# HKUST-Aerial-Robotics/Omni-swarm

Measured on AMD Instinct MI355X. Metric: keyframes/sec (4x fisheye 600x480) + p50 loop-match ms @ 100k-frame DB, higher is better.
Workload: dtype f16

## Files before the change

omni-swarm_amd/csrc/config.h:

```cpp
#pragma once
#include "common.h"

namespace omni {

enum CfgId {
    CFG_CONV_V1 = 0, CFG_RS_TRN, CFG_DET16, CFG_SP_SPARSE_DESC, CFG_SP_SPARSE_DA, CFG_SP_FUSED_CAND, CFG_SP_SPLIT_DB, CFG_SP_MASK_SKIP, CFG_SP_MASK_SKIP_SPLIT, CFG_SP_MASK_RECT, CFG_SPLIT_FUSE1A, CFG_SPLIT_WINO,
    CFG_SPLIT_TRN, CFG_CONV_XCD, CFG_SP_PROFILE_MASK, CFG_PP_U8, CFG_PP_TRACE, CFG_PP_DBG, CFG_RS_TRACE, CFG_SPLIT_TRACE, CFG_SPLIT_DBG, CFG_WINO_TRACE, CFG_ROCTX,
    CFG_VLAD_BIG, CFG_VLAD_STEM_FUSE, CFG_VLAD_UNFUSED, CFG_VLAD_MFMA, CFG_VLAD_SBLOCK, CFG_VLAD_MBLOCK_PX, CFG_VLAD_MFMA_PX, CFG_VLAD_FC_MFMA, CFG_VLAD_MBLOCK_CPW,
    CFG_VLAD_SB_LDSPAD, CFG_VLAD_SB_PERSIST, CFG_VLAD_SB_TRACE, CFG_VLAD_SB_DBG, CFG_VLAD_MASK_SKIP,
    CFG_SCAN_ROWS_MIN, CFG_MQ_ROT, CFG_MQ_MIN, CFG_INDEX_MIRROR, CFG_INDEX_MIRROR_MIN_ROWS, CFG_INDEX_CERT_FAIL,
    CFG_GEOMETRY_THREADS, CFG_MESSAGE_THREADS, CFG_GEOMETRY_ASYNC, CFG_DETECTOR_ASYNC, CFG_PIPELINE_ONE_STREAM, CFG_PIPELINE_FIFO, CFG_PIPELINE_UNIT_PLAN,
    CFG_JPEGDEC_SUBSEQ_BITS, CFG_JPEGDEC_RESTART_WGS, CFG_JPEGDEC_PLAIN_WGS, CFG_JPEGDEC_UNSTUFF_DEV,
    CFG_HW_QUEUES,
    CFG_RCCL_LIB,
    CFG_COUNT
};
enum CfgClass {
    CFG_VARIANT = 0,
    CFG_TUNING = 1,
    CFG_DEBUG = 2,
    CFG_TEST = 3,
    CFG_STRING = 4
};
struct CfgOption { const char* env; int def, lo, hi; int cls; const char* doc; };
// ... 13 lines not shown
```

omni-swarm_amd/csrc/config.hip:

```cpp
#include "config.h"
#include "stream_plan.h"

#include <atomic>
#include <cerrno>
#include <climits>
#include <cstdlib>

namespace omni {

const CfgOption kCfgOptions[CFG_COUNT] = {
    {"OMNI_CONV_V1", 0, 0, 3, CFG_VARIANT, "fp16 3x3 layers: 0 = production (conv1a fused into the ping-pong conv1b, register-stationary cin=128); 1 = generic kernel, 2 = persistent LDS-DMA kernel, "
                                           "3 = ping-pong without the conv1a fusion -- 1-3 exist only in the test build of the library (lib_test/)"},
    {"OMNI_RS_TRN", -1, -1, 1, CFG_VARIANT, "register-stationary kernel of the unpooled cin=128 fp16 layers: tile orientation, -1 = the one with fewer tiles, 0 = plain, 1 = transposed"},
    {"OMNI_DET16", 1, 0, 1, CFG_VARIANT, "detector head of the fp16 and OMNI_PREC_SPLIT paths on v_mfma_f32_32x32x16_f16 with split (hi, lo) operands (0: the exact-f32 MFMA kernel)"},
    {"OMNI_SP_SPARSE_DESC", 1, 0, 1, CFG_VARIANT, "convDb + descriptor norm only at the cells around the key points (0: dense descriptor map)"},
    {"OMNI_SP_SPARSE_DA", 1, 0, 1, CFG_VARIANT, "convDa only at those cells too (fp16 and OMNI_PREC_SPLIT; 0: dense convDa)"},
    {"OMNI_SP_FUSED_CAND", 1, 0, 1, CFG_VARIANT, "getKeyPoints' threshold inside the detector head's epilogue + window masks from the candidate list (0: sp_cand_kernel re-reads the heat map)"},
    {"OMNI_SP_SPLIT_DB", 1, 0, 1, CFG_VARIANT, "OMNI_PREC_SPLIT: convDb + descriptor norm at the key points' cells with split (hi, lo) operands on the fp16 matrix cores (0: exact-f32 MFMA convolution)"},
    {"OMNI_SP_MASK_SKIP", 1, 0, 1, CFG_VARIANT, "fp16: the tile rows inside the image-independent band of the fisheye mask are left out of the tile walk (0: every tile)"},
    {"OMNI_SP_MASK_SKIP_SPLIT", 1, 0, 1, CFG_VARIANT, "the same for OMNI_PREC_SPLIT"},
    {"OMNI_SP_MASK_RECT", 0, 0, 1, CFG_TEST, "1: a masked pass leaves out only the rectangle of tiles where the output is one constant vector, filled by broadcasting that vector "
                                             "(what was skipped before the band: the A/B reference, same results)"},
    {"OMNI_SPLIT_FUSE1A", 1, 0, 1, CFG_VARIANT, "OMNI_PREC_SPLIT: conv1a built inside the conv1b kernel from the u8 image (0: separate exact-f32 conv1a pass)"},
    {"OMNI_SPLIT_WINO", 7, 0, 15, CFG_VARIANT, "OMNI_PREC_SPLIT: the cin = 64 layers as Winograd F(2x2,3x3) kernels with split operands (conv_wino.hip), bit 0 = conv1b (with the conv1a "
                                                "fusion), 1 = conv2a, 2 = conv2b, 3 = conv3a (off by default: same time as the direct kernel, profiles/r06g); 0: the direct kernels of conv_split.hip"},
    {"OMNI_SPLIT_TRN", -1, -1, 1, CFG_VARIANT, "OMNI_PREC_SPLIT cin=128 kernel: tile orientation, as OMNI_RS_TRN"},
    {"OMNI_CONV_XCD", 1, 0, 1, CFG_VARIANT, "persistent convolution kernels derive (cout group, tile walk) from an XCD-aware block id: the cout groups of a pixel tile and its neighbours "
                                           "share one L2 (0: plain blockIdx; process-wide, same results either way)"},
    {"OMNI_SP_PROFILE_MASK", 0, 0, 1, CFG_TUNING, "omni_sp_profile times the stages with the fisheye mask on (what the key-frame pipeline runs)"},
    {"OMNI_PP_U8", 1, 0, 1, CFG_VARIANT, "fp16 conv1a inside conv1b's kernel: matrix-core operands straight from the image bytes (0: through the 256-entry u8 -> (hi, lo) table in LDS)"},
    {"OMNI_PP_TRACE", 0, 0, 1, CFG_DEBUG, "s_memtime trace of the ping-pong conv kernel on stderr"},
    {"OMNI_PP_DBG", 0, 0, 255, CFG_DEBUG, "ping-pong conv kernel timing ablations (WRONG results)"},
    {"OMNI_RS_TRACE", 0, 0, 1, CFG_DEBUG, "s_memtime trace of the register-stationary kernel"},
    {"OMNI_SPLIT_TRACE", 0, 0, 1, CFG_DEBUG, "s_memtime trace of the split-precision kernel"},
    {"OMNI_SPLIT_DBG", 0, 0, 3, CFG_DEBUG, "split-precision kernel timing ablations: 1 = no stores, 2 = every DMA reads tile 0 (WRONG results)"},
    {"OMNI_WINO_TRACE", 0, 0, 1, CFG_DEBUG, "s_memtime trace of the Winograd split kernel"},
    {"OMNI_ROCTX", 0, 0, 1, CFG_DEBUG, "roctx ranges around upload / SuperPoint / MobileNetVLAD / post-processing / BF match / index add + search / exchange and the host loop's "
                                      "stages (rocprofv3 --marker-trace; the library is resolved by dlopen)"},
    {"OMNI_VLAD_BIG", 0, 0, 128, CFG_TUNING, "64 / 128: the 64- / 128-pixel tiles of the unfused block kernel (measured slower at 600x480)"},
    {"OMNI_VLAD_STEM_FUSE", 1, 0, 1, CFG_VARIANT, "stem + block 0 in one kernel (0: two kernels)"},
    {"OMNI_VLAD_UNFUSED", 0, 0, 1, CFG_VARIANT, "1: every block as expand / depthwise / project launches"},
    {"OMNI_VLAD_MFMA", 1, 0, 1, CFG_VARIANT, "late blocks' 1x1 convolutions on the matrix cores"},
    {"OMNI_VLAD_SBLOCK", 1, 0, 1, CFG_VARIANT, "fused split-fp16 block kernel (vlad_s.hip)"},
    {"OMNI_VLAD_MBLOCK_PX", 2048, 0, 1 << 24, CFG_TUNING, "fused matrix-core block kernel for blocks of at most this many input pixels per image (0 disables)"},
    {"OMNI_VLAD_MFMA_PX", 0, 0, 1 << 24, CFG_TUNING, "> 0: matrix-core 1x1 convolutions for blocks of at most this many input pixels per image (default 2048)"},
// ... 138 lines not shown
```

omni-swarm_amd/csrc/conv.h:

```cpp
#pragma once
#include "common.h"
#include "tile_walk.h"

namespace omni {

#define CONV_TH 8
#define CONV_TW 32
#define RS_TH 6
#define RS_TW 32
int conv_rs_pool_tile_rows();
#define CONV_COUT_TILE 64
#define CONV_CIN_CHUNK 64

static inline size_t conv_packed_elems(int cin, int cout, int ksize) { return (size_t)cin * cout * ksize * ksize; }

void conv_pack_weights_f16(const float* w_oihw, int cin, int cout, int ksize, __half* out);
void conv_pack_weights_f32(const float* w_oihw, int cin, int cout, int ksize, float* out);

struct ConvArgs {
    const void* in;
    void* out;
    const void* w_packed;
    const float* bias;
    int batch, H, W, cin, cout, ksize;
// ... 23 lines not shown
void conv1a_split_pack_fused(const float* w , const float* bias , uint16_t* frag );
int conv1ab_split_fused(hipStream_t stream, const ConvArgs& a, const uint8_t* gray, int gstride, int fisheye_mask, const void* w1a_frag, const uint32_t* lut_hl);
float conv_pack_weights_wino(const float* w_oihw, int cin, int cout, uint16_t* out);
int conv_wino(hipStream_t stream, const ConvArgs& a, bool out_split);
int conv1ab_wino_fused(hipStream_t stream, const ConvArgs& a, const uint8_t* gray, int gstride, int fisheye_mask, const void* w1a_frag, const uint32_t* lut_hl, bool out_split);
int split_to_raw32(hipStream_t stream, const void* in_split, void* out_raw, int batch, int C, int H, int W);
int conv_read_pixels2x2_bytes(hipStream_t stream, const void* map, int64_t row_bytes, int64_t org_bytes, int pix_bytes, int y, int x, void* vec);
int conv_fill_rect2x2_bytes(hipStream_t stream, void* map, int batch, int64_t img_bytes, int64_t row_bytes, int64_t org_bytes, int pix_bytes, int y0, int y1, int x0, int x1,
                            const void* vec);
int raw32_to_nchw_f32(hipStream_t stream, const void* in_raw, float* out, int batch, int C, int H, int W);
__host__ __device__ inline int split_frame_w(int W) { return ((W + 31) & ~31) + 2; }
__host__ __device__ inline int split_frame_h(int H) { return ((H + 31) & ~31) + 2; }
inline size_t split_frame_bytes(int H, int W, int C) { return (size_t)split_frame_h(H) * split_frame_w(W) * C * 4; }

int conv1ab_fused(hipStream_t stream, const ConvArgs& a, const uint8_t* gray, int gstride, int fisheye_mask, const _Float16* w1a_frag,
                  const float* bias1a, const uint32_t* lut_hl);
void conv1a_pack_split_weights(const float* w , const float* bias , uint16_t* frag );
void conv1a_make_split_lut(uint32_t* lut );
void conv1a_pack_u8_weights(const float* w , const float* bias , uint16_t* frag );

int conv1a_direct(hipStream_t stream, int precision, const uint8_t* gray, int stride, int batch, int H, int W,
                  int fisheye_mask, const float* w, const float* bias, const float* u8_lut, void* out);

int detector_head(hipStream_t stream, int precision, const void* in, int in_stride, int in_off, int batch, int Hc, int Wc,
                  const float* wT, const float* bias, float* semi);

#if defined(__HIPCC__)
__device__ __forceinline__ int xcd_block_id(int enable) {
    const int n = (int)gridDim.x, b = (int)blockIdx.x;
    return (enable && (n & 7) == 0) ? (b & 7) * (n >> 3) + (b >> 3) : b;
}
// ... 31 lines not shown
```

omni-swarm_amd/csrc/conv.hip:

```cpp
#include "config.h"
#include "conv.h"
#include <type_traits>

namespace omni {

typedef _Float16 half8_t __attribute__((ext_vector_type(8)));
typedef _Float16 half4_t __attribute__((ext_vector_type(4)));
typedef float floatx16 __attribute__((ext_vector_type(16)));
typedef float floatx4 __attribute__((ext_vector_type(4)));

template <typename T, int KG, int EPL>
static void pack_weights(const float* w, int cin, int cout, int ks, T* out) {
    const int taps = ks * ks, n_ct = cout / 64, n_ch = cin / 64;
    size_t o = 0;
    for (int ct = 0; ct < n_ct; ++ct)
        for (int ch = 0; ch < n_ch; ++ch)
            for (int tap = 0; tap < taps; ++tap)
                for (int kg = 0; kg < KG; ++kg)
                    for (int m = 0; m < 2; ++m)
                        for (int l = 0; l < 64; ++l)
                            for (int e = 0; e < EPL; ++e) {
                                const int co = ct * 64 + m * 32 + (l & 31);
                                const int ci = ch * 64 + kg * (64 / KG) + (l >> 5) * EPL + e;
                                const float v = w[((size_t)co * cin + ci) * taps + tap];
// ... 394 lines not shown
        const uint32_t addr = bb[ky + (WHICH == 3 ? 1 : 0)][kx] ^ (kg << 5);
        asm volatile("ds_read_b128 %0, %1" : "=v"(dst) : "v"(addr));
    } else {
        constexpr int aoff = (STEP % 18) * 2048 + (WHICH == 2 ? 1024 : 0);
        const uint32_t ab = STEP < 18 ? a_base0 : a_base1;
        asm volatile("ds_read_b128 %0, %1 offset:%2" : "=v"(dst) : "v"(ab), "i"(aoff));
    }
}
template <int STEP>
__device__ __forceinline__ void pp_load_step(uint32_t a_base0, uint32_t a_base1, const uint32_t (&bb)[4][3], half8_t& fa0, half8_t& fa1,
                                             half8_t& fb0, half8_t& fb1) {
    pp_read<STEP, 0>(a_base0, a_base1, bb, fb0);
    pp_read<STEP, 1>(a_base0, a_base1, bb, fa0);
    pp_read<STEP, 2>(a_base0, a_base1, bb, fa1);
    pp_read<STEP, 3>(a_base0, a_base1, bb, fb1);
}

template <int N>
__device__ __forceinline__ void pp_wait(half8_t& fa0, half8_t& fa1, half8_t& fb0, half8_t& fb1) {
    asm volatile("s_waitcnt lgkmcnt(%4)" : "+v"(fa0), "+v"(fa1), "+v"(fb0), "+v"(fb1) : "i"(N));
}

template <int STEP, int ABL>
__device__ __forceinline__ void pp_mfma_steps(uint32_t a_base0, uint32_t a_base1, const uint32_t (&bb)[4][3], floatx16 (&acc)[2][2],
                                              half8_t (&fa0)[3], half8_t (&fa1)[3], half8_t (&fb0)[3], half8_t (&fb1)[3]) {
    if constexpr (STEP < 36) {
        constexpr int sl = STEP % 3, nx = (STEP + 2) % 3;
        constexpr bool pre = STEP + 2 < 36;
        constexpr bool rdB = pre && ABL != 1 && ABL != 2, rdA = pre && ABL != 1 && ABL != 3;
        pp_wait<ABL ? 0 : ((STEP + 1 < 36) ? 4 : 0)>(fa0[sl], fa1[sl], fb0[sl], fb1[sl]);
// ... 17 lines not shown
        pp_mfma_steps<STEP + 1, ABL>(a_base0, a_base1, bb, acc, fa0, fa1, fb0, fb1);
    }
}

struct Fuse1aArgs {
    const uint8_t* gray; int gstride; int mask_r0, mask_r1;
    const _Float16* w1a_frag;
    const float* bias1a;
    const uint32_t* lut_hl;
    unsigned long long* trace;
    const char* zero_page;
    uint32_t magic_tpi;
    TileWalk walk;
};

template <bool POOL, int ABL, bool FUSE1A>
__global__ void __launch_bounds__(PP_THREADS)
conv3x3_c64_pp_kernel(const _Float16* __restrict__ in, _Float16* __restrict__ out, const _Float16* __restrict__ wp,
                      const float* __restrict__ bias, int H, int W, int cout, int n_ct, int tiles_x, int tiles_y, int batch, int relu, int dbg,
                      Fuse1aArgs fz) {
    extern __shared__ __attribute__((aligned(16))) char smem_raw[];
    const uint32_t lds0 = (uint32_t)(uintptr_t)(__attribute__((address_space(3))) char*)smem_raw;
    const int tid = threadIdx.x, lane = tid & 63;
    const int wave = __builtin_amdgcn_readfirstlane(tid >> 6);
    const int grp = wave >> 2, wl = wave & 3;
    const int n = lane & 31, hh = lane >> 5;
    const int bid = xcd_block_id(fz.walk.xcd);
    const int ct = bid % n_ct, wg = bid / n_ct, nwg = gridDim.x / n_ct;
    const int total = batch * fz.walk.act;
    const int n_mine = wg < total ? (total - wg + nwg - 1) / nwg : 0;

    {
        const uint4* src = reinterpret_cast<const uint4*>(wp + (int64_t)ct * 9 * 4096);
        uint4* dst = reinterpret_cast<uint4*>(smem_raw);
        for (int i = tid; i < C64_W_BYTES / 16; i += PP_THREADS) dst[i] = src[i];
    }
    constexpr int BUFB = FUSE1A ? C64_PIX * 128 : C64_BUF_BYTES;
    char* const buf = smem_raw + C64_W_BYTES + grp * BUFB;
    const uint32_t buf_lds = lds0 + C64_W_BYTES + grp * BUFB;
    uint32_t bb[4][3];
#pragma unroll
    for (int r = 0; r < 4; ++r)
#pragma unroll
        for (int kx = 0; kx < 3; ++kx) {
            const int p = (2 * wl + r) * C64_ITW + n + kx;
            bb[r][kx] = buf_lds + p * 128 + ((hh ^ ((p >> 1) & 7)) << 4);
        }
    const uint32_t a_base0 = lds0 + lane * 16, a_base1 = a_base0 + 18 * 2048;

    auto tile_origin = [&](int t, int& b, int& ty0, int& tx0) {
        b = tile_walk_div(t, fz.magic_tpi);
        int ry, rx;
        tile_walk_rc(fz.walk, tiles_x, t - b * fz.walk.act, ry, rx);
        ty0 = ry * CONV_TH; tx0 = rx * CONV_TW;
// ... 56 lines not shown
        const int p = (3 * wl + fi) * 32 + n;
        fr_iy[fi] = p / C64_ITW; fr_ix[fi] = p - fr_iy[fi] * C64_ITW;
    }
    unsigned char* const patch = reinterpret_cast<unsigned char*>(lut_lds + 256) + wl * 240;
    int tap_off[5];
#pragma unroll
    for (int k = 0; k < 5; ++k) { const int tp = hh ? (k < 4 ? 5 + k : 8) : k; tap_off[k] = (tp / 3) * 40 + tp % 3; }
    auto build_issue = [&](int b, int ty0, int tx0, uint32_t& pv) {
        const int j = lane / 10, d = lane - j * 10;
        int yy = ty0 - 2 + fr_r0 + j, xo = ((tx0 - 2) & ~3) + 4 * d;
        yy = yy < 0 ? 0 : (yy >= H ? H - 1 : yy);
        xo = xo < 0 ? 0 : (xo > fz.gstride - 4 ? fz.gstride - 4 : xo);
        const auto rsrc = __builtin_amdgcn_make_buffer_rsrc(const_cast<uint8_t*>(fz.gray), 0, batch * H * fz.gstride, 0x00020000);
        pv = __builtin_amdgcn_raw_buffer_load_b32(rsrc, (b * H + yy) * fz.gstride + xo, 0, 0);
    };
    auto build_finish = [&](int b, int ty0, int tx0, uint32_t pv, unsigned long long* stamp = nullptr) {
        (void)b;
        const int cx0 = (tx0 - 2) & ~3, xsh = (tx0 - 2) - cx0;
        {
            const int j = lane / 10, d = lane - j * 10;
            const int yy = ty0 - 2 + fr_r0 + j, x0c = cx0 + 4 * d;
            const bool rok = yy >= 0 && yy < H && !(yy >= fz.mask_r0 && yy < fz.mask_r1);
            uint32_t bm = 0;
#pragma unroll
            for (int k = 0; k < 4; ++k) bm |= (x0c + k >= 0 && x0c + k < W) ? (0xFFu << (8 * k)) : 0u;
            if (lane < 60) reinterpret_cast<uint32_t*>(patch)[lane] = rok ? (pv & bm) : 0u;
        }
        half8_t wa[2][2];
#pragma unroll
        for (int j = 0; j < 2; ++j)
#pragma unroll
// ... 33 lines not shown
        for (int fi = 0; fi < 3; ++fi) {
            if (fi >= nf) continue;
#pragma unroll
            for (int m = 0; m < 2; ++m) {
#pragma unroll
                for (int i = 0; i < 16; ++i) a1[fi][m][i] = 0.f;
                a1[fi][m] = __builtin_amdgcn_mfma_f32_32x32x16_f16(wa[0][m], B0[fi], a1[fi][m], 0, 0, 0);
            }
        }
#pragma unroll
        for (int fi = 0; fi < 3; ++fi) {
            if (fi >= nf) continue;
#pragma unroll
            for (int m = 0; m < 2; ++m) a1[fi][m] = __builtin_amdgcn_mfma_f32_32x32x16_f16(wa[1][m], B1[fi], a1[fi][m], 0, 0, 0);
        }
        __builtin_amdgcn_s_setprio(0);
        if (stamp) stamp[1] = __builtin_amdgcn_s_memtime();
#pragma unroll
        for (int fi = 0; fi < 3; ++fi) {
            if (fi >= nf) continue;
            const int p = (3 * wl + fi) * 32 + n;
            const uint32_t sw = (uint32_t)((p >> 1) & 7);
            char* const prow = buf + p * 128 + 8 * hh;
            if (p < C64_PIX) {
#pragma unroll
                for (int m = 0; m < 2; ++m)
#pragma unroll
                    for (int gq = 0; gq < 4; ++gq)
                        *reinterpret_cast<uint2*>(prow + (((uint32_t)(m * 4 + gq) ^ sw) << 4)) =
                            make_uint2(pack_relu_f16(a1[fi][m][4 * gq + 0], a1[fi][m][4 * gq + 1], 1), pack_relu_f16(a1[fi][m][4 * gq + 2], a1[fi][m][4 * gq + 3], 1));
            }
        }
    };

    int k_load = grp;
    int ob = 0, oty0 = 0, otx0 = 0;
    __syncthreads();
    if (grp == 0 && k_load < n_mine) {
        tile_origin(wg + k_load * nwg, ob, oty0, otx0);
        if constexpr (FUSE1A) {
            uint32_t pv;
            build_issue(ob, oty0, otx0, pv);
            build_finish(ob, oty0, otx0, pv);
        } else {
            issue(ob, oty0, otx0);
            asm volatile("s_waitcnt vmcnt(0)" ::: "memory");
        }
        k_load += 2;
    }
    __syncthreads();

    floatx16 acc[2][2];
    int t_pending = -1;
    for (int p = 0; p <= n_mine; ++p) {
        if ((p & 1) == grp) {
            if (p < n_mine) {
#pragma unroll
                for (int m = 0; m < 2; ++m)
#pragma unroll
                    for (int f = 0; f < 2; ++f)
#pragma unroll
                        for (int i = 0; i < 16; ++i) acc[m][f][i] = 0.f;
#pragma unroll
                for (int r = 0; r < 4; ++r)
#pragma unroll
                    for (int kx = 0; kx < 3; ++kx) asm volatile("" : "+v"(bb[r][kx]));
                half8_t fa0[3], fa1[3], fb0[3], fb1[3];
                pp_load_step<0>(a_base0, a_base1, bb, fa0[0], fa1[0], fb0[0], fb1[0]);
                pp_load_step<1>(a_base0, a_base1, bb, fa0[1], fa1[1], fb0[1], fb1[1]);
                __builtin_amdgcn_sched_barrier(0);
                if (!(dbg & 16)) __builtin_amdgcn_s_setprio(2);
                const bool trc = fz.trace && blockIdx.x == 0 && wl == 0 && lane == 0 && p >= 2 && p < 6;
                if (trc) fz.trace[p * 8 + 4] = __builtin_amdgcn_s_memtime();
                pp_mfma_steps<0, ABL>(a_base0, a_base1, bb, acc, fa0, fa1, fb0, fb1);
                if (trc) fz.trace[p * 8 + 5] = __builtin_amdgcn_s_memtime();
                __builtin_amdgcn_s_setprio(0);
                t_pending = wg + p * nwg;
            }
        } else {
            float4 bs[POOL ? 1 : 2][4];
            if constexpr (POOL) bias4(n & 1, bs[0]);
            else { bias4(0, bs[0]); bias4(1, bs[1]); }
            __builtin_amdgcn_sched_barrier(0);
            const bool load = k_load < n_mine && !(dbg & 1);
            if (dbg & 32) __builtin_amdgcn_s_setprio(3);
            uint32_t pv = 0;
            const bool tr = fz.trace && blockIdx.x == 0 && wl == 0 && lane == 0 && p >= 2 && p < 6;
            if (tr) fz.trace[p * 8 + 0] = __builtin_amdgcn_s_memtime();
            int nb = 0, nty0 = 0, ntx0 = 0;
            if (load) {
                tile_origin(wg + k_load * nwg, nb, nty0, ntx0);
                if constexpr (FUSE1A) build_issue(nb, nty0, ntx0, pv);
                else issue(nb, nty0, ntx0);
            }
            if (tr) fz.trace[p * 8 + 1] = __builtin_amdgcn_s_memtime();
            bool full = false;
            if (t_pending >= 0 && !(dbg & 2)) {
                const int b = ob, ty0 = oty0, tx0 = otx0;
                full = (ty0 + CONV_TH <= H) && (tx0 + CONV_TW <= W);
                const int ox = tx0 + n;
                if constexpr (POOL) {
                    const int oy = ty0 + 2 * wl;
                    const bool odd = n & 1;
                    float v[16], q0[16], q1[16];
#pragma unroll
                    for (int i = 0; i < 16; ++i) { q0[i] = vmax(acc[0][0][i], acc[0][1][i]); q1[i] = vmax(acc[1][0][i], acc[1][1][i]); }
                    __builtin_amdgcn_sched_barrier(0);
#pragma unroll
                    for (int i = 0; i < 16; ++i) {
                        const float h0 = vmax_swap_pairs(q0[i]), h1 = vmax_swap_pairs(q1[i]);
                        v[i] = odd ? h1 : h0;
                    }
// ... 5 lines not shown
                        const int oy = ty0 + 2 * wl + f;
#pragma unroll
                        for (int m = 0; m < 2; ++m) {
                            float v[16];
#pragma unroll
                            for (int i = 0; i < 16; ++i) v[i] = acc[m][f][i];
                            _Float16* o = out + (((int64_t)b * H + oy) * W + ox) * cout + ct * 64 + m * 32;
                            store_frag16<false>(v, bs[m], o, hh, relu, (oy < H) && (ox < W));
                        }
                    }
                }
                t_pending = -1;
            }
            if (tr) fz.trace[p * 8 + 2] = __builtin_amdgcn_s_memtime();
            if (load && FUSE1A) {
                if constexpr (FUSE1A) build_finish(nb, nty0, ntx0, pv, tr ? fz.trace + p * 8 + 6 : nullptr);
                if (tr) fz.trace[p * 8 + 3] = __builtin_amdgcn_s_memtime();
                k_load += 2;
                ob = nb; oty0 = nty0; otx0 = ntx0;
            } else if (load) {
                if (full) {
                    if constexpr (POOL) asm volatile("s_waitcnt vmcnt(2)" ::: "memory");
                    else asm volatile("s_waitcnt vmcnt(8)" ::: "memory");
                } else {
                    asm volatile("s_waitcnt vmcnt(0)" ::: "memory");
                }
                if (tr) fz.trace[p * 8 + 3] = __builtin_amdgcn_s_memtime();
                k_load += 2;
                ob = nb; oty0 = nty0; otx0 = ntx0;
            }
        }
        if (dbg & 32) __builtin_amdgcn_s_setprio(0);
        asm volatile("s_waitcnt lgkmcnt(0)" ::: "memory");
        __builtin_amdgcn_s_barrier();
    }
}

template <bool POOL, int ABL, bool FUSE1A = false>
static int launch_conv_pp_abl(hipStream_t st, const ConvArgs& a, int n_cu, int dbg, const Fuse1aArgs& fz = Fuse1aArgs{}) {
    auto kfn = conv3x3_c64_pp_kernel<POOL, ABL, FUSE1A>;
    constexpr int smem_bytes = FUSE1A ? PP_SMEM_FUSED : PP_SMEM;
    static_assert(smem_bytes <= 160 * 1024, "LDS budget");
    OMNI_HIP_TRY(hipFuncSetAttribute((const void*)kfn, hipFuncAttributeMaxDynamicSharedMemorySize, smem_bytes));
    const int tiles_x = cdiv(a.W, CONV_TW), tiles_y = cdiv(a.H, CONV_TH), n_ct = a.cout / 64;
    Fuse1aArgs fzz = fz;
    if (int rc = tile_walk_plan(fzz.walk, "conv", tiles_x, tiles_y, a.skip_ty0, a.skip_ty1, a.skip_tx0, a.skip_tx1)) return rc;
    fzz.walk.xcd = config_process()[CFG_CONV_XCD];
    const int total = a.batch * fzz.walk.act;
    const int per_ct = tile_walk_grid(n_cu, n_ct, cdiv(total, 2));
    OMNI_REQUIRE(a.zero_page, OMNI_ERR_INVALID, "conv: ConvArgs.zero_page is not set");
    fzz.zero_page = reinterpret_cast<const char*>(a.zero_page);
    OMNI_REQUIRE((int64_t)total * (tiles_x * tiles_y) < (1ll << 32), OMNI_ERR_INVALID, "conv: too many tiles for the multiply-high division");
    fzz.magic_tpi = tile_walk_magic(fzz.walk.act);
    static const bool want_trace = config_process()[CFG_PP_TRACE] != 0;
    static unsigned long long* trace_dev = nullptr;
    if (want_trace && !FUSE1A) {
        if (!trace_dev) OMNI_HIP_TRY(hipMalloc((void**)&trace_dev, 64 * 8));
        OMNI_HIP_TRY(hipMemsetAsync(trace_dev, 0, 64 * 8, st));
        fzz.trace = trace_dev;
    }
    hipLaunchKernelGGL(kfn, dim3(per_ct * n_ct), dim3(PP_THREADS), smem_bytes, st, reinterpret_cast<const _Float16*>(a.in),
                       reinterpret_cast<_Float16*>(a.out), reinterpret_cast<const _Float16*>(a.w_packed), a.bias, a.H, a.W, a.cout, n_ct,
                       tiles_x, tiles_y, a.batch, a.relu ? 1 : 0, dbg, fzz);
    OMNI_LAUNCH_CHECK();
    if (want_trace && !FUSE1A) {
        unsigned long long h[64];
        OMNI_HIP_TRY(hipMemcpyAsync(h, trace_dev, sizeof(h), hipMemcpyDeviceToHost, st));
        OMNI_HIP_TRY(hipStreamSynchronize(st));
        static int launches = 0;
        if (total >= 16 * per_ct && launches++ < 2)
            for (int p = 2; p < 6; ++p)
                if (h[p * 8])
                    fprintf(stderr, "pp trace pool=%d H=%d W=%d cout=%d phase %d: service: issue %llu epilogue %llu dma wait %llu | partner mfma loop %llu\n", (int)POOL, a.H, a.W,
                            a.cout, p, h[p * 8 + 1] - h[p * 8], h[p * 8 + 2] - h[p * 8 + 1], h[p * 8 + 3] - h[p * 8 + 2], h[(p ^ 1) * 8 + 5] - h[(p ^ 1) * 8 + 4]);
    }
    return OMNI_OK;
// ... 582 lines not shown
}

template <typename T, int KS, bool POOL>
static int launch_conv(hipStream_t st, const ConvArgs& a) {
    const size_t smem = conv_smem_bytes<T, KS>();
    auto kfn = conv_mfma_kernel<T, KS, POOL>;
    OMNI_HIP_TRY(hipFuncSetAttribute((const void*)kfn, hipFuncAttributeMaxDynamicSharedMemorySize, (int)smem));
    dim3 grid(cdiv(a.W, CONV_TW) * cdiv(a.H, CONV_TH), a.cout / CONV_COUT_TILE, a.batch);
    hipLaunchKernelGGL(kfn, grid, dim3(256), smem, st, reinterpret_cast<const T*>(a.in), a.out, reinterpret_cast<const T*>(a.w_packed),
                       a.bias, a.H, a.W, a.cin, a.cout, a.relu ? 1 : 0, a.out_f32 ? 1 : 0, a.in_cstride > 0 ? a.in_cstride : a.cin);
    OMNI_LAUNCH_CHECK();
    return OMNI_OK;
}

int conv1ab_fused(hipStream_t st, const ConvArgs& a, const uint8_t* gray, int gstride, int fisheye_mask, const _Float16* w1a_frag,
                  const float* bias1a, const uint32_t* lut_hl) {
    OMNI_REQUIRE(a.cin == 64 && a.cout % 64 == 0 && a.ksize == 3 && a.pool && a.n_cu > 0, OMNI_ERR_INVALID, "conv1ab_fused: bad layer shape");
    OMNI_REQUIRE(gstride % 4 == 0 && ((uintptr_t)gray & 3) == 0 && (int64_t)a.batch * a.H * gstride < (1ll << 31), OMNI_ERR_INVALID,
                 "conv1ab_fused: image rows must be 4-byte aligned (stride %d)", gstride);
    Fuse1aArgs fz;
    fz.gray = gray; fz.gstride = gstride;
    omni_fisheye_mask_rows(a.H, fisheye_mask, &fz.mask_r0, &fz.mask_r1);
    fz.w1a_frag = w1a_frag; fz.bias1a = bias1a; fz.lut_hl = lut_hl; fz.trace = nullptr;
    static const bool want_trace = config_process()[CFG_PP_TRACE] != 0;
    static unsigned long long* trace_dev = nullptr;
    if (want_trace) {
        if (!trace_dev) OMNI_HIP_TRY(hipMalloc((void**)&trace_dev, 64 * 8));
        OMNI_HIP_TRY(hipMemsetAsync(trace_dev, 0, 64 * 8, st));
        fz.trace = trace_dev;
    }
    static const int dbg = config_process()[CFG_PP_DBG];
    const int rc = launch_conv_pp_abl<true, 0, true>(st, a, a.n_cu, dbg, fz);
    if (want_trace && rc == OMNI_OK) {
        unsigned long long h[64];
        OMNI_HIP_TRY(hipMemcpyAsync(h, trace_dev, sizeof(h), hipMemcpyDeviceToHost, st));
        OMNI_HIP_TRY(hipStreamSynchronize(st));
        static int printed = 0;
        if (printed++ == 20)
            for (int p = 2; p < 6; ++p)
                fprintf(stderr, "pp trace phase %d: service start %llu issue +%llu epilogue +%llu build +%llu (operands ready +%llu, first fragment +%llu) | mfma loop %llu cycles (start +%lld vs service start)\n", p,
                        h[p * 8], h[p * 8 + 1] - h[p * 8], h[p * 8 + 2] - h[p * 8 + 1], h[p * 8 + 3] - h[p * 8 + 2], h[p * 8 + 6] - h[p * 8 + 2], h[p * 8 + 7] - h[p * 8 + 6],
                        h[p * 8 + 5] - h[p * 8 + 4], (long long)(h[p * 8 + 4] - h[p * 8]));
    }
    return rc;
}

static inline uint16_t f2h_bits(float v) { const __half h = __float2half_rn(v); uint16_t u; memcpy(&u, &h, 2); return u; }
static inline float h2f(uint16_t u) { __half h; memcpy(&h, &u, 2); return __half2float(h); }
void conv1a_pack_split_weights(const float* w, const float* bias, uint16_t* frag ) {
    for (int j = 0; j < 2; ++j)
        for (int m = 0; m < 2; ++m)
            for (int l = 0; l < 64; ++l)
                for (int e = 0; e < 8; ++e) {
                    const int co = m * 32 + (l & 31), hh = l >> 5;
                    auto hi = [&](int t) { return f2h_bits(w[co * 9 + t]); };
                    auto lo = [&](int t) { return f2h_bits(w[co * 9 + t] - h2f(f2h_bits(w[co * 9 + t]))); };
                    uint16_t v = 0;
// ... 938 lines not shown
```

omni-swarm_amd/csrc/sp_plan.h:

```cpp
#pragma once
#include "../../include/omni_hip.h"

namespace omni {

struct SpHandleFacts {
    int precision = OMNI_PREC_F32, H = 0, W = 0;
    int conv_variant = 0;
    bool det16 = true;
    bool fused_cand = true;
    bool sparse_desc = true;
    bool sparse_da = true;
    bool split_fuse1a = true;
    bool split_db = true;
    int wino = 0;
    bool mask_skip = false;
};

inline int sp_wino_layers(int precision, int requested, int H, int W, bool split_fuse1a) {
    if (precision != OMNI_PREC_SPLIT) return 0;
    int m = requested;
    if (H % 8 != 0 || W % 8 != 0) m &= 7;
    if (H % 4 != 0 || W % 4 != 0) m &= 1;
    if (H % 2 != 0 || W % 2 != 0 || !split_fuse1a) m &= ~1;
    return m;
}

struct SpPassInputs {
// ... 13 lines not shown
    SP_DESC_GATHER_F32,
    SP_DESC_SPARSE_DA_SPLIT,
};

struct SpC64Plan {
    bool wino = false;
    bool convert_in = false;
    bool out_raw32 = false;
};

struct SpPassPlan {
    bool calibrating = false;
    SpConv1a conv1a = SP_1A_DIRECT;
    SpConv1b conv1b = SP_1B_CONV;
    bool raw_1b = false;
    SpC64Plan conv2a, conv2b, conv3a;
    bool use_skip = false;
    bool heads_sparse_da = false;
    bool tails_f32 = true;
    SpDetTail det = SP_DET_MFMA_F32;
    bool cand_fused = false;
    SpDescTail desc = SP_DESC_DENSE_GENERIC;
    bool desc_split_db = false;
    bool run_post = false;
    bool dense_valid = false;
    bool heads_full = true;
};

inline SpPassPlan sp_plan_pass(const SpHandleFacts& f, const SpPassInputs& in) {
    const bool f16 = f.precision == OMNI_PREC_F16, split = f.precision == OMNI_PREC_SPLIT, best = f.conv_variant == 0;
    SpPassPlan p;
    p.calibrating = in.calibrating; p.run_post = in.run_post;
    const bool fuse1a = ((f16 && best) || (split && f.split_fuse1a)) && in.aligned4;
    p.conv1a = fuse1a ? SP_1A_FUSED : split ? SP_1A_SPLIT : SP_1A_DIRECT;
    const int wino = split ? f.wino : 0;
    p.conv1b = !fuse1a ? SP_1B_CONV : !split ? SP_1B_FUSED_F16 : (wino & 1) ? SP_1B_FUSED_WINO : SP_1B_FUSED_SPLIT;
    const bool w[4] = {p.conv1b == SP_1B_FUSED_WINO, (wino & 2) != 0, (wino & 4) != 0, (wino & 8) != 0};
    SpC64Plan* c64[3] = {&p.conv2a, &p.conv2b, &p.conv3a};
    p.raw_1b = w[0] && w[1];
    for (int i = 0; i < 3; ++i) {
        c64[i]->wino = w[i + 1];
        c64[i]->convert_in = w[i + 1] && !w[i];
        c64[i]->out_raw32 = w[i + 1] && i < 2 && w[i + 2];
    }
    p.use_skip = f.mask_skip && in.fisheye_mask && (fuse1a || split) && !in.calibrating;
    const bool sparse = best && f.sparse_desc && in.run_post;
    const bool sparse_da = sparse && f.sparse_da && (f16 || split);
    p.heads_sparse_da = sparse_da;
    p.tails_f32 = !f16;
    p.det = f.conv_variant == 1 ? SP_DET_VALU : (f16 && f.det16) ? SP_DET_MFMA16_F16 : (split && f.det16) ? SP_DET_MFMA16_F32 : SP_DET_MFMA_F32;
    p.cand_fused = in.run_post && f.fused_cand && f.conv_variant != 1;
    p.desc = sparse ? (f16 ? (sparse_da ? SP_DESC_SPARSE_DA_F16 : SP_DESC_SPARSE_F16) : (sparse_da ? SP_DESC_SPARSE_DA_SPLIT : SP_DESC_GATHER_F32))
                    : (f16 && best) ? SP_DESC_DENSE_F16 : SP_DESC_DENSE_GENERIC;
    p.desc_split_db = p.desc == SP_DESC_SPARSE_DA_SPLIT && f.split_db;
// ... 21 lines not shown
```

omni-swarm_amd/csrc/superpoint.hip:

```cpp
#include <algorithm>
#include <vector>

#include "config.h"
#include "conv.h"
#include "sp_plan.h"
#include "sp_post.h"

namespace {
struct LayerDef { const char* name; int cin, cout, ks, div; bool pool; };
const LayerDef kLayers[OMNI_SP_NUM_LAYERS] = {
    {"conv1a", 1, 64, 3, 1, false},    {"conv1b", 64, 64, 3, 1, true},     {"conv2a", 64, 64, 3, 2, false},    {"conv2b", 64, 64, 3, 2, true},
    {"conv3a", 64, 128, 3, 4, false},  {"conv3b", 128, 128, 3, 4, true},   {"conv4a", 128, 128, 3, 8, false},  {"conv4b", 128, 128, 3, 8, false},
    {"convPa", 128, 256, 3, 8, false}, {"convPb", 256, 65, 1, 8, false},   {"convDa", 128, 256, 3, 8, false},  {"convDb", 256, 256, 1, 8, false}};
enum { L1A = 0, L1B, L2A, L2B, L3A, L3B, L4A, L4B, LPA, LPB, LDA, LDB };
enum { ST_CONV1A = 0, ST_CONV1B, ST_CONV2A, ST_CONV2B, ST_CONV3A, ST_CONV3B, ST_CONV4A, ST_CONV4B, ST_HEADS_A,
       ST_DET_TAIL, ST_DESC_TAIL, ST_POST, ST_COUNT };
const char* kStageNames[OMNI_SP_NUM_STAGES] = {
    "conv1a", "conv1b+pool", "conv2a", "conv2b+pool", "conv3a", "conv3b+pool", "conv4a", "conv4b", "convPa|convDa",
    "convPb+softmax+d2s", "convDb+l2norm", "nms+topk+describe", "", "", "", ""};
}

struct omni_sp {
    omni_ctx* ctx = nullptr;
    omni::Config cfg;
// ... 138 lines not shown
        }
    }
    return OMNI_OK;
}

static void sp_set_facts(omni_sp* s) {
    SpHandleFacts& f = s->facts;
    f.precision = s->precision; f.H = s->H; f.W = s->W;
    f.conv_variant = s->cfg[CFG_CONV_V1];
    f.det16 = s->cfg[CFG_DET16] != 0;
    f.fused_cand = s->cfg[CFG_SP_FUSED_CAND] != 0;
    f.sparse_desc = s->cfg[CFG_SP_SPARSE_DESC] != 0;
    f.sparse_da = s->cfg[CFG_SP_SPARSE_DA] != 0;
    f.split_fuse1a = s->cfg[CFG_SPLIT_FUSE1A] != 0;
    f.split_db = s->cfg[CFG_SP_SPLIT_DB] != 0;
    f.wino = sp_wino_layers(s->precision, s->cfg[CFG_SPLIT_WINO], s->H, s->W, f.split_fuse1a);
}

static int sp_init(omni_sp* s, const omni_sp_weights* w, const float* pca_comp, const float* pca_mean) {
    hipStream_t st = s->ctx->stream;
    int rc;
    for (int l = 0; l < OMNI_SP_NUM_LAYERS; ++l)
        if ((rc = dev_upload(s, &s->bias[l], w->bias[l], (size_t)kLayers[l].cout * 4))) return rc;
    if ((rc = dev_upload(s, &s->w1a, w->weight[L1A], 64 * 9 * 4))) return rc;
    {
        std::vector<float> t(256 * 65);
        for (int c = 0; c < 65; ++c)
            for (int k = 0; k < 256; ++k) t[(size_t)k * 65 + c] = w->weight[LPB][(size_t)c * 256 + k];
        if ((rc = dev_upload(s, &s->wPbT, t.data(), t.size() * 4))) return rc;
        std::vector<float> wa(16384), wdst(256);
// ... 235 lines not shown
    s->skip_state = step.after;
    s->last = p; s->last_batch = batch;
    auto mark = [&]() -> int { if (with_events) OMNI_HIP_TRY(hipEventRecord(s->ev[stage], st)); ++stage; return OMNI_OK; };
    if ((rc = mark())) return rc;
    switch (p.conv1a) {
        case SP_1A_FUSED: break;
        case SP_1A_SPLIT: rc = conv1a_split(st, gray_dev, stride, batch, H, W, fisheye_mask, s->w1a, s->bias[L1A], s->lut, s->a1a, p.use_skip ? s->mskip[0].ty0 : 0, p.use_skip ? s->mskip[0].ty1 : 0); break;
        case SP_1A_DIRECT: rc = conv1a_direct(st, s->precision, gray_dev, stride, batch, H, W, fisheye_mask, s->w1a, s->bias[L1A], s->lut, s->a1a); break;
    }
    if (rc || (rc = mark())) return rc;
    if (p.conv1b == SP_1B_CONV) rc = sp_conv(s, p, L1B, s->a1a, s->a1b, batch);
    else {
        const ConvArgs a = sp_layer_args(s, p, L1B, p.conv1b == SP_1B_FUSED_WINO ? SP_K_WINO : SP_K_DIRECT, nullptr, s->a1b, batch);
        if (p.conv1b == SP_1B_FUSED_WINO) rc = conv1ab_wino_fused(st, a, gray_dev, stride, fisheye_mask, s->w1a_frag, s->lut_hl, !p.raw_1b);
        else if (p.conv1b == SP_1B_FUSED_SPLIT) rc = conv1ab_split_fused(st, a, gray_dev, stride, fisheye_mask, s->w1a_frag, s->lut_hl);
        else rc = conv1ab_fused(st, a, gray_dev, stride, fisheye_mask, reinterpret_cast<const _Float16*>(s->w1a_frag), s->bias[L1A], s->lut_hl);
    }
    if (rc || (rc = mark())) return rc;
    auto c64 = [&](int l, const SpC64Plan& c, const void* in, void* out) -> int {
        if (!c.wino) return sp_conv(s, p, l, in, out, batch);
        if (c.convert_in) {
            if (!s->a_tmp && (rc = s->mem.alloc(&s->a_tmp, (size_t)s->max_batch * split_frame_bytes(H / 2, W / 2, 64)))) return rc;
            if ((rc = split_to_raw32(st, in, s->a_tmp, batch, 64, H / kLayers[l].div, W / kLayers[l].div))) return rc;
            in = s->a_tmp;
        }
        return conv_wino(st, sp_layer_args(s, p, l, SP_K_WINO, in, out, batch), !c.out_raw32);
    };
    if ((rc = c64(L2A, p.conv2a, s->a1b, s->a2a)) || (rc = mark())) return rc;
    if ((rc = c64(L2B, p.conv2b, s->a2a, s->a2b)) || (rc = mark())) return rc;
    if ((rc = c64(L3A, p.conv3a, s->a2b, s->a3a)) || (rc = mark())) return rc;
    if ((rc = sp_conv(s, p, L3B, s->a3a, s->a3b, batch)) || (rc = mark())) return rc;
// ... 412 lines not shown
```

Measured before the change: 2680.

## Add third builder wave group to fused conv1a/conv1b ping-pong kernel

Adds a three-role variant of the fused conv1a+conv1b ping-pong kernel with 768 threads. A dedicated builder group constructs the conv1a halo tiles into alternating LDS buffers while one group runs MFMAs and the other runs the epilogue, and barriers keep the three in step. This takes halo building off the epilogue group's critical path. It also merges the step-0/1 LDS operand loads into one asm block. The cost is more threads per workgroup, which may lower occupancy or raise register pressure, and an extra tile_origin recomputation in the epilogue.

```diff
diff --git a/omni-swarm_amd/csrc/config.h b/omni-swarm_amd/csrc/config.h
--- a/omni-swarm_amd/csrc/config.h
+++ b/omni-swarm_amd/csrc/config.h
@@ -5,7 +5,7 @@
 
 enum CfgId {
     CFG_CONV_V1 = 0, CFG_RS_TRN, CFG_DET16, CFG_SP_SPARSE_DESC, CFG_SP_SPARSE_DA, CFG_SP_FUSED_CAND, CFG_SP_SPLIT_DB, CFG_SP_MASK_SKIP, CFG_SP_MASK_SKIP_SPLIT, CFG_SP_MASK_RECT, CFG_SPLIT_FUSE1A, CFG_SPLIT_WINO,
-    CFG_SPLIT_TRN, CFG_CONV_XCD, CFG_SP_PROFILE_MASK, CFG_PP_U8, CFG_PP_TRACE, CFG_PP_DBG, CFG_RS_TRACE, CFG_SPLIT_TRACE, CFG_SPLIT_DBG, CFG_WINO_TRACE, CFG_ROCTX,
+    CFG_SPLIT_TRN, CFG_CONV_XCD, CFG_SP_PROFILE_MASK, CFG_PP_U8, CFG_PP_BUILDERS, CFG_PP_TRACE, CFG_PP_DBG, CFG_RS_TRACE, CFG_SPLIT_TRACE, CFG_SPLIT_DBG, CFG_WINO_TRACE, CFG_ROCTX,
     CFG_VLAD_BIG, CFG_VLAD_STEM_FUSE, CFG_VLAD_UNFUSED, CFG_VLAD_MFMA, CFG_VLAD_SBLOCK, CFG_VLAD_MBLOCK_PX, CFG_VLAD_MFMA_PX, CFG_VLAD_FC_MFMA, CFG_VLAD_MBLOCK_CPW,
     CFG_VLAD_SB_LDSPAD, CFG_VLAD_SB_PERSIST, CFG_VLAD_SB_TRACE, CFG_VLAD_SB_DBG, CFG_VLAD_MASK_SKIP,
     CFG_SCAN_ROWS_MIN, CFG_MQ_ROT, CFG_MQ_MIN, CFG_INDEX_MIRROR, CFG_INDEX_MIRROR_MIN_ROWS, CFG_INDEX_CERT_FAIL,
diff --git a/omni-swarm_amd/csrc/config.hip b/omni-swarm_amd/csrc/config.hip
--- a/omni-swarm_amd/csrc/config.hip
+++ b/omni-swarm_amd/csrc/config.hip
@@ -29,6 +29,8 @@
                                            "share one L2 (0: plain blockIdx; process-wide, same results either way)"},
     {"OMNI_SP_PROFILE_MASK", 0, 0, 1, CFG_TUNING, "omni_sp_profile times the stages with the fisheye mask on (what the key-frame pipeline runs)"},
     {"OMNI_PP_U8", 1, 0, 1, CFG_VARIANT, "fp16 conv1a inside conv1b's kernel: matrix-core operands straight from the image bytes (0: through the 256-entry u8 -> (hi, lo) table in LDS)"},
+    {"OMNI_PP_BUILDERS", 1, 0, 1, CFG_TUNING, "fp16 conv1a inside conv1b's kernel: 1 = three wave groups, 768 threads, the third builds the conv1a halo tiles while one group runs its MFMA loop "
+                                              "and the other its epilogue; 0 = two groups of 512 threads, the idle one does both (the A/B reference; same bytes either way)"},
     {"OMNI_PP_TRACE", 0, 0, 1, CFG_DEBUG, "s_memtime trace of the ping-pong conv kernel on stderr"},
     {"OMNI_PP_DBG", 0, 0, 255, CFG_DEBUG, "ping-pong conv kernel timing ablations (WRONG results)"},
     {"OMNI_RS_TRACE", 0, 0, 1, CFG_DEBUG, "s_memtime trace of the register-stationary kernel"},
diff --git a/omni-swarm_amd/csrc/conv.h b/omni-swarm_amd/csrc/conv.h
--- a/omni-swarm_amd/csrc/conv.h
+++ b/omni-swarm_amd/csrc/conv.h
@@ -61,7 +61,7 @@
 inline size_t split_frame_bytes(int H, int W, int C) { return (size_t)split_frame_h(H) * split_frame_w(W) * C * 4; }
 
 int conv1ab_fused(hipStream_t stream, const ConvArgs& a, const uint8_t* gray, int gstride, int fisheye_mask, const _Float16* w1a_frag,
-                  const float* bias1a, const uint32_t* lut_hl);
+                  const float* bias1a, const uint32_t* lut_hl, int builders);
 void conv1a_pack_split_weights(const float* w , const float* bias , uint16_t* frag );
 void conv1a_make_split_lut(uint32_t* lut );
 void conv1a_pack_u8_weights(const float* w , const float* bias , uint16_t* frag );
diff --git a/omni-swarm_amd/csrc/conv.hip b/omni-swarm_amd/csrc/conv.hip
--- a/omni-swarm_amd/csrc/conv.hip
+++ b/omni-swarm_amd/csrc/conv.hip
@@ -432,6 +432,15 @@
     pp_read<STEP, 1>(a_base0, a_base1, bb, fa0);
     pp_read<STEP, 2>(a_base0, a_base1, bb, fa1);
     pp_read<STEP, 3>(a_base0, a_base1, bb, fb1);
+}
+
+__device__ __forceinline__ void pp_load_steps01(uint32_t a_base0, const uint32_t (&bb)[4][3], half8_t (&fa0)[3], half8_t (&fa1)[3], half8_t (&fb0)[3],
+                                                half8_t (&fb1)[3]) {
+    const uint32_t b0 = bb[0][0], b1 = bb[1][0], b0k = b0 ^ 32, b1k = b1 ^ 32;
+    asm volatile("ds_read_b128 %0, %8\n\tds_read_b128 %1, %12\n\tds_read_b128 %2, %12 offset:1024\n\tds_read_b128 %3, %9\n\t"
+                 "ds_read_b128 %4, %10\n\tds_read_b128 %5, %12 offset:2048\n\tds_read_b128 %6, %12 offset:3072\n\tds_read_b128 %7, %11"
+                 : "=&v"(fb0[0]), "=&v"(fa0[0]), "=&v"(fa1[0]), "=&v"(fb1[0]), "=&v"(fb0[1]), "=&v"(fa0[1]), "=&v"(fa1[1]), "=&v"(fb1[1])
+                 : "v"(b0), "v"(b1), "v"(b0k), "v"(b1k), "v"(a_base0));
 }
 
 template <int N>
@@ -479,8 +488,8 @@
     TileWalk walk;
 };
 
-template <bool POOL, int ABL, bool FUSE1A>
-__global__ void __launch_bounds__(PP_THREADS)
+template <bool POOL, int ABL, bool FUSE1A, int ROLES = 2>
+__global__ void __launch_bounds__(ROLES * 256)
 conv3x3_c64_pp_kernel(const _Float16* __restrict__ in, _Float16* __restrict__ out, const _Float16* __restrict__ wp,
                       const float* __restrict__ bias, int H, int W, int cout, int n_ct, int tiles_x, int tiles_y, int batch, int relu, int dbg,
                       Fuse1aArgs fz) {
@@ -488,6 +497,7 @@
     const uint32_t lds0 = (uint32_t)(uintptr_t)(__attribute__((address_space(3))) char*)smem_raw;
     const int tid = threadIdx.x, lane = tid & 63;
     const int wave = __builtin_amdgcn_readfirstlane(tid >> 6);
+    static_assert(ROLES == 2 || (ROLES == 3 && FUSE1A), "the builder group builds conv1a halo tiles");
     const int grp = wave >> 2, wl = wave & 3;
     const int n = lane & 31, hh = lane >> 5;
     const int bid = xcd_block_id(fz.walk.xcd);
@@ -498,11 +508,11 @@
     {
         const uint4* src = reinterpret_cast<const uint4*>(wp + (int64_t)ct * 9 * 4096);
         uint4* dst = reinterpret_cast<uint4*>(smem_raw);
-        for (int i = tid; i < C64_W_BYTES / 16; i += PP_THREADS) dst[i] = src[i];
+        for (int i = tid; i < C64_W_BYTES / 16; i += ROLES * 256) dst[i] = src[i];
     }
     constexpr int BUFB = FUSE1A ? C64_PIX * 128 : C64_BUF_BYTES;
-    char* const buf = smem_raw + C64_W_BYTES + grp * BUFB;
-    const uint32_t buf_lds = lds0 + C64_W_BYTES + grp * BUFB;
+    char* const buf = smem_raw + C64_W_BYTES + (grp & 1) * BUFB;
+    const uint32_t buf_lds = lds0 + C64_W_BYTES + (grp & 1) * BUFB;
     uint32_t bb[4][3];
 #pragma unroll
     for (int r = 0; r < 4; ++r)
@@ -589,7 +599,7 @@
         const auto rsrc = __builtin_amdgcn_make_buffer_rsrc(const_cast<uint8_t*>(fz.gray), 0, batch * H * fz.gstride, 0x00020000);
         pv = __builtin_amdgcn_raw_buffer_load_b32(rsrc, (b * H + yy) * fz.gstride + xo, 0, 0);
     };
-    auto build_finish = [&](int b, int ty0, int tx0, uint32_t pv, unsigned long long* stamp = nullptr) {
+    auto build_finish = [&](int b, int ty0, int tx0, uint32_t pv, char* const wbuf, unsigned long long* stamp = nullptr) {
         (void)b;
         const int cx0 = (tx0 - 2) & ~3, xsh = (tx0 - 2) - cx0;
         {
@@ -653,14 +663,15 @@
 #pragma unroll
             for (int m = 0; m < 2; ++m) a1[fi][m] = __builtin_amdgcn_mfma_f32_32x32x16_f16(wa[1][m], B1[fi], a1[fi][m], 0, 0, 0);
         }
-        __builtin_amdgcn_s_setprio(0);
+        if (ROLES == 3 && (dbg & 64)) __builtin_amdgcn_s_setprio(1);
+        else __builtin_amdgcn_s_setprio(0);
         if (stamp) stamp[1] = __builtin_amdgcn_s_memtime();
 #pragma unroll
         for (int fi = 0; fi < 3; ++fi) {
             if (fi >= nf) continue;
             const int p = (3 * wl + fi) * 32 + n;
             const uint32_t sw = (uint32_t)((p >> 1) & 7);
-            char* const prow = buf + p * 128 + 8 * hh;
+            char* const prow = wbuf + p * 128 + 8 * hh;
             if (p < C64_PIX) {
 #pragma unroll
                 for (int m = 0; m < 2; ++m)
@@ -672,15 +683,15 @@
         }
     };
 
-    int k_load = grp;
+    int k_load = ROLES == 3 ? 0 : grp;
     int ob = 0, oty0 = 0, otx0 = 0;
     __syncthreads();
-    if (grp == 0 && k_load < n_mine) {
+    if ((ROLES == 3 ? grp == 2 : grp == 0) && k_load < n_mine) {
         tile_origin(wg + k_load * nwg, ob, oty0, otx0);
         if constexpr (FUSE1A) {
             uint32_t pv;
             build_issue(ob, oty0, otx0, pv);
-            build_finish(ob, oty0, otx0, pv);
+            build_finish(ob, oty0, otx0, pv, smem_raw + C64_W_BYTES);
         } else {
             issue(ob, oty0, otx0);
             asm volatile("s_waitcnt vmcnt(0)" ::: "memory");
@@ -691,6 +702,27 @@
 
     floatx16 acc[2][2];
     int t_pending = -1;
+    if constexpr (ROLES == 3) {
+        if (grp == 2) {
+            if (dbg & 64) __builtin_amdgcn_s_setprio(1);
+            for (int p = 0; p <= n_mine; ++p) {
+                const bool tr = fz.trace && blockIdx.x == 0 && wl == 0 && lane == 0 && p >= 2 && p < 6;
+                if (tr) fz.trace[p * 8 + 0] = __builtin_amdgcn_s_memtime();
+                if (p + 1 < n_mine && !(dbg & 1)) {
+                    int nb, nty0, ntx0;
+                    uint32_t pv;
+                    tile_origin(wg + (p + 1) * nwg, nb, nty0, ntx0);
+                    build_issue(nb, nty0, ntx0, pv);
+                    if (tr) fz.trace[p * 8 + 1] = __builtin_amdgcn_s_memtime();
+                    build_finish(nb, nty0, ntx0, pv, smem_raw + C64_W_BYTES + ((p + 1) & 1) * BUFB, tr ? fz.trace + p * 8 + 6 : nullptr);
+                    if (tr) fz.trace[p * 8 + 3] = __builtin_amdgcn_s_memtime();
+                }
+                asm volatile("s_waitcnt lgkmcnt(0)" ::: "memory");
+                __builtin_amdgcn_s_barrier();
+            }
+            return;
+        }
+    }
     for (int p = 0; p <= n_mine; ++p) {
         if ((p & 1) == grp) {
             if (p < n_mine) {
@@ -705,8 +737,11 @@
 #pragma unroll
                     for (int kx = 0; kx < 3; ++kx) asm volatile("" : "+v"(bb[r][kx]));
                 half8_t fa0[3], fa1[3], fb0[3], fb1[3];
-                pp_load_step<0>(a_base0, a_base1, bb, fa0[0], fa1[0], fb0[0], fb1[0]);
-                pp_load_step<1>(a_base0, a_base1, bb, fa0[1], fa1[1], fb0[1], fb1[1]);
+                if constexpr (ROLES == 3 && ABL == 0) pp_load_steps01(a_base0, bb, fa0, fa1, fb0, fb1);
+                else {
+                    pp_load_step<0>(a_base0, a_base1, bb, fa0[0], fa1[0], fb0[0], fb1[0]);
+                    pp_load_step<1>(a_base0, a_base1, bb, fa0[1], fa1[1], fb0[1], fb1[1]);
+                }
                 __builtin_amdgcn_sched_barrier(0);
                 if (!(dbg & 16)) __builtin_amdgcn_s_setprio(2);
                 const bool trc = fz.trace && blockIdx.x == 0 && wl == 0 && lane == 0 && p >= 2 && p < 6;
@@ -721,20 +756,21 @@
             if constexpr (POOL) bias4(n & 1, bs[0]);
             else { bias4(0, bs[0]); bias4(1, bs[1]); }
             __builtin_amdgcn_sched_barrier(0);
-            const bool load = k_load < n_mine && !(dbg & 1);
+            const bool load = ROLES == 2 && k_load < n_mine && !(dbg & 1);
             if (dbg & 32) __builtin_amdgcn_s_setprio(3);
             uint32_t pv = 0;
             const bool tr = fz.trace && blockIdx.x == 0 && wl == 0 && lane == 0 && p >= 2 && p < 6;
-            if (tr) fz.trace[p * 8 + 0] = __builtin_amdgcn_s_memtime();
+            if (tr) fz.trace[ROLES == 3 ? 64 + p : p * 8 + 0] = __builtin_amdgcn_s_memtime();
             int nb = 0, nty0 = 0, ntx0 = 0;
             if (load) {
                 tile_origin(wg + k_load * nwg, nb, nty0, ntx0);
                 if constexpr (FUSE1A) build_issue(nb, nty0, ntx0, pv);
                 else issue(nb, nty0, ntx0);
             }
-            if (tr) fz.trace[p * 8 + 1] = __builtin_amdgcn_s_memtime();
+            if (tr && ROLES == 2) fz.trace[p * 8 + 1] = __builtin_amdgcn_s_memtime();
             bool full = false;
             if (t_pending >= 0 && !(dbg & 2)) {
+                if constexpr (ROLES == 3) tile_origin(t_pending, ob, oty0, otx0);
                 const int b = ob, ty0 = oty0, tx0 = otx0;
                 full = (ty0 + CONV_TH <= H) && (tx0 + CONV_TW <= W);
                 const int ox = tx0 + n;
@@ -770,7 +806,7 @@
             }
             if (tr) fz.trace[p * 8 + 2] = __builtin_amdgcn_s_memtime();
             if (load && FUSE1A) {
-                if constexpr (FUSE1A) build_finish(nb, nty0, ntx0, pv, tr ? fz.trace + p * 8 + 6 : nullptr);
+                if constexpr (FUSE1A) build_finish(nb, nty0, ntx0, pv, buf, tr ? fz.trace + p * 8 + 6 : nullptr);
                 if (tr) fz.trace[p * 8 + 3] = __builtin_amdgcn_s_memtime();
                 k_load += 2;
                 ob = nb; oty0 = nty0; otx0 = ntx0;
@@ -792,9 +828,9 @@
     }
 }
 
-template <bool POOL, int ABL, bool FUSE1A = false>
+template <bool POOL, int ABL, bool FUSE1A = false, int ROLES = 2>
 static int launch_conv_pp_abl(hipStream_t st, const ConvArgs& a, int n_cu, int dbg, const Fuse1aArgs& fz = Fuse1aArgs{}) {
-    auto kfn = conv3x3_c64_pp_kernel<POOL, ABL, FUSE1A>;
+    auto kfn = conv3x3_c64_pp_kernel<POOL, ABL, FUSE1A, ROLES>;
     constexpr int smem_bytes = FUSE1A ? PP_SMEM_FUSED : PP_SMEM;
     static_assert(smem_bytes <= 160 * 1024, "LDS budget");
     OMNI_HIP_TRY(hipFuncSetAttribute((const void*)kfn, hipFuncAttributeMaxDynamicSharedMemorySize, smem_bytes));
@@ -815,7 +851,7 @@
         OMNI_HIP_TRY(hipMemsetAsync(trace_dev, 0, 64 * 8, st));
         fzz.trace = trace_dev;
     }
-    hipLaunchKernelGGL(kfn, dim3(per_ct * n_ct), dim3(PP_THREADS), smem_bytes, st, reinterpret_cast<const _Float16*>(a.in),
+    hipLaunchKernelGGL(kfn, dim3(per_ct * n_ct), dim3(ROLES * 256), smem_bytes, st, reinterpret_cast<const _Float16*>(a.in),
                        reinterpret_cast<_Float16*>(a.out), reinterpret_cast<const _Float16*>(a.w_packed), a.bias, a.H, a.W, a.cout, n_ct,
                        tiles_x, tiles_y, a.batch, a.relu ? 1 : 0, dbg, fzz);
     OMNI_LAUNCH_CHECK();
@@ -1428,7 +1464,7 @@
 }
 
 int conv1ab_fused(hipStream_t st, const ConvArgs& a, const uint8_t* gray, int gstride, int fisheye_mask, const _Float16* w1a_frag,
-                  const float* bias1a, const uint32_t* lut_hl) {
+                  const float* bias1a, const uint32_t* lut_hl, int builders) {
     OMNI_REQUIRE(a.cin == 64 && a.cout % 64 == 0 && a.ksize == 3 && a.pool && a.n_cu > 0, OMNI_ERR_INVALID, "conv1ab_fused: bad layer shape");
     OMNI_REQUIRE(gstride % 4 == 0 && ((uintptr_t)gray & 3) == 0 && (int64_t)a.batch * a.H * gstride < (1ll << 31), OMNI_ERR_INVALID,
                  "conv1ab_fused: image rows must be 4-byte aligned (stride %d)", gstride);
@@ -1439,22 +1475,29 @@
     static const bool want_trace = config_process()[CFG_PP_TRACE] != 0;
     static unsigned long long* trace_dev = nullptr;
     if (want_trace) {
-        if (!trace_dev) OMNI_HIP_TRY(hipMalloc((void**)&trace_dev, 64 * 8));
-        OMNI_HIP_TRY(hipMemsetAsync(trace_dev, 0, 64 * 8, st));
+        if (!trace_dev) OMNI_HIP_TRY(hipMalloc((void**)&trace_dev, 128 * 8));
+        OMNI_HIP_TRY(hipMemsetAsync(trace_dev, 0, 128 * 8, st));
         fz.trace = trace_dev;
     }
     static const int dbg = config_process()[CFG_PP_DBG];
-    const int rc = launch_conv_pp_abl<true, 0, true>(st, a, a.n_cu, dbg, fz);
+    const int rc = builders ? launch_conv_pp_abl<true, 0, true, 3>(st, a, a.n_cu, dbg, fz) : launch_conv_pp_abl<true, 0, true, 2>(st, a, a.n_cu, dbg, fz);
     if (want_trace && rc == OMNI_OK) {
-        unsigned long long h[64];
+        unsigned long long h[128];
         OMNI_HIP_TRY(hipMemcpyAsync(h, trace_dev, sizeof(h), hipMemcpyDeviceToHost, st));
         OMNI_HIP_TRY(hipStreamSynchronize(st));
         static int printed = 0;
         if (printed++ == 20)
-            for (int p = 2; p < 6; ++p)
+            for (int p = 2; p < 6; ++p) {
+                if (builders)
+                    fprintf(stderr, "pp trace phase %d: builder start %llu issue +%llu operands ready +%llu mfmas issued +%llu done +%llu (= %llu cycles) | epilogue %llu cycles "
+                                    "(start %+lld vs builder) | mfma loop %llu cycles (start %+lld vs builder)\n", p,
+                            h[p * 8], h[p * 8 + 1] - h[p * 8], h[p * 8 + 6] - h[p * 8 + 1], h[p * 8 + 7] - h[p * 8 + 6], h[p * 8 + 3] - h[p * 8 + 7], h[p * 8 + 3] - h[p * 8],
+                            h[p * 8 + 2] - h[64 + p], (long long)(h[64 + p] - h[p * 8]), h[p * 8 + 5] - h[p * 8 + 4], (long long)(h[p * 8 + 4] - h[p * 8]));
+                else
                 fprintf(stderr, "pp trace phase %d: service start %llu issue +%llu epilogue +%llu build +%llu (operands ready +%llu, first fragment +%llu) | mfma loop %llu cycles (start +%lld vs service start)\n", p,
                         h[p * 8], h[p * 8 + 1] - h[p * 8], h[p * 8 + 2] - h[p * 8 + 1], h[p * 8 + 3] - h[p * 8 + 2], h[p * 8 + 6] - h[p * 8 + 2], h[p * 8 + 7] - h[p * 8 + 6],
                         h[p * 8 + 5] - h[p * 8 + 4], (long long)(h[p * 8 + 4] - h[p * 8]));
+            }
     }
     return rc;
 }
diff --git a/omni-swarm_amd/csrc/sp_plan.h b/omni-swarm_amd/csrc/sp_plan.h
--- a/omni-swarm_amd/csrc/sp_plan.h
+++ b/omni-swarm_amd/csrc/sp_plan.h
@@ -11,6 +11,7 @@
     bool sparse_desc = true;
     bool sparse_da = true;
     bool split_fuse1a = true;
+    bool pp_builders = true;
     bool split_db = true;
     int wino = 0;
     bool mask_skip = false;
@@ -54,6 +55,7 @@
     SpConv1a conv1a = SP_1A_DIRECT;
     SpConv1b conv1b = SP_1B_CONV;
     bool raw_1b = false;
+    bool builders_1b = false;
     SpC64Plan conv2a, conv2b, conv3a;
     bool use_skip = false;
     bool heads_sparse_da = false;
@@ -78,6 +80,7 @@
     const bool w[4] = {p.conv1b == SP_1B_FUSED_WINO, (wino & 2) != 0, (wino & 4) != 0, (wino & 8) != 0};
     SpC64Plan* c64[3] = {&p.conv2a, &p.conv2b, &p.conv3a};
     p.raw_1b = w[0] && w[1];
+    p.builders_1b = p.conv1b == SP_1B_FUSED_F16 && f.pp_builders;
     for (int i = 0; i < 3; ++i) {
         c64[i]->wino = w[i + 1];
         c64[i]->convert_in = w[i + 1] && !w[i];
diff --git a/omni-swarm_amd/csrc/superpoint.hip b/omni-swarm_amd/csrc/superpoint.hip
--- a/omni-swarm_amd/csrc/superpoint.hip
+++ b/omni-swarm_amd/csrc/superpoint.hip
@@ -176,6 +176,7 @@
     f.sparse_da = s->cfg[CFG_SP_SPARSE_DA] != 0;
     f.split_fuse1a = s->cfg[CFG_SPLIT_FUSE1A] != 0;
     f.split_db = s->cfg[CFG_SP_SPLIT_DB] != 0;
+    f.pp_builders = s->cfg[CFG_PP_BUILDERS] != 0;
     f.wino = sp_wino_layers(s->precision, s->cfg[CFG_SPLIT_WINO], s->H, s->W, f.split_fuse1a);
 }
 
@@ -441,7 +442,7 @@
         const ConvArgs a = sp_layer_args(s, p, L1B, p.conv1b == SP_1B_FUSED_WINO ? SP_K_WINO : SP_K_DIRECT, nullptr, s->a1b, batch);
         if (p.conv1b == SP_1B_FUSED_WINO) rc = conv1ab_wino_fused(st, a, gray_dev, stride, fisheye_mask, s->w1a_frag, s->lut_hl, !p.raw_1b);
         else if (p.conv1b == SP_1B_FUSED_SPLIT) rc = conv1ab_split_fused(st, a, gray_dev, stride, fisheye_mask, s->w1a_frag, s->lut_hl);
-        else rc = conv1ab_fused(st, a, gray_dev, stride, fisheye_mask, reinterpret_cast<const _Float16*>(s->w1a_frag), s->bias[L1A], s->lut_hl);
+        else rc = conv1ab_fused(st, a, gray_dev, stride, fisheye_mask, reinterpret_cast<const _Float16*>(s->w1a_frag), s->bias[L1A], s->lut_hl, p.builders_1b ? 1 : 0);
     }
     if (rc || (rc = mark())) return rc;
     auto c64 = [&](int l, const SpC64Plan& c, const void* in, void* out) -> int {
```

Result: no change. 2673 (-0.3%).
